# haoosz/FFR-Net

Hardware: AMD Instinct MI355X
Metric: face embeddings/sec (IR-SE50 + RecNet forward, 112x112 fp32) at batch 256 per GPU (higher is better)
Workload: dtype f32; 1 GPU; configs[2]: IR-SE50 + RecBlock (spatial+channel) forward, batch 256 per GPU, 112x112x3 fp32 -> f_new,f [512]; + all-gather of embeddings and pair cosine scores (112x96 of the BASELINE label cannot be embedded by the reference: BASELINE.md); batch_per_gpu=256, global_batch=256, parallelism=image-sharded x1, RCCL all-gather of embeddings

## Files before the change

ffr-net_amd/csrc/elementwise.hip:

```cpp
#include "device_util.h"
#include "ffr_kernels.h"

namespace ffr {

#define STEM_PIX 64
#define STEM_STEPS 8
#define STEM_TLD 36
template <bool U8>
__global__ __launch_bounds__(256) void k_stem(const float* __restrict__ x, const unsigned char* __restrict__ xu8,
                                             const unsigned char* __restrict__ flip, const float* __restrict__ w,
                                             const float* __restrict__ bias, const float* __restrict__ slope,
                                             float* __restrict__ out, int N, int H, int W,
                                             const float* __restrict__ x2, int n_split,
                                             const unsigned char* __restrict__ xu8b) {
    __shared__ __attribute__((aligned(16))) float patch[STEM_PIX * 28];
    __shared__ __attribute__((aligned(16))) float otile[4 * 32 * STEM_TLD];
    __shared__ float lut[U8 ? 257 : 1];
    const int tid = threadIdx.x;
    if constexpr (U8) {
        lut[tid] = __fdiv_rn(__fsub_rn(__fdiv_rn((float)tid, 255.0f), 0.5f), 0.5f);
        if (tid == 0) lut[256] = 0.f;
    }
    const int lane = tid & 63, wave = tid >> 6;
    const int mt = wave >> 1, nt = wave & 1;
// ... 270 lines not shown
                          int N, int Ho, int Wo, int C, int stride, hipStream_t stream) {
    const long long total4 = (long long)N * Ho * Wo * (C >> 2);
    const int cq = C >> 2;
    int shift = 0;
    while ((1 << shift) < cq) ++shift;
    if ((1 << shift) != cq || total4 >= 0x7fffffffLL || C % 4) return hipErrorInvalidValue;
    unsigned blocks = (unsigned)((total4 + 255) / 256);
    if (blocks > 8192) blocks = 8192;
    hipLaunchKernelGGL(k_combine, dim3(blocks), dim3(256), 0, stream, res, scale, sc, x, out, (unsigned)(Ho * Wo), (unsigned)Wo, C, stride,
                       (unsigned)total4, shift);
    return hipGetLastError();
}

__global__ __launch_bounds__(256) void k_affine(const float* __restrict__ x, const float* __restrict__ s,
                                               const float* __restrict__ t, float* __restrict__ y, int C,
                                               long long total4) {
    const int cq = C >> 2;
    for (long long idx = (long long)blockIdx.x * 256 + threadIdx.x; idx < total4; idx += (long long)gridDim.x * 256) {
        const int c4 = (int)(idx % cq) * 4;
        const f32x4 v = *reinterpret_cast<const f32x4*>(x + idx * 4);
        const f32x4 sv = *reinterpret_cast<const f32x4*>(s + c4);
        const f32x4 tv = *reinterpret_cast<const f32x4*>(t + c4);
        *reinterpret_cast<f32x4*>(y + idx * 4) = v * sv + tv;
    }
}

hipError_t launch_affine(const float* x, const float* s, const float* t, float* y, int M, int C, hipStream_t stream) {
    const long long total4 = (long long)M * (C >> 2);
    unsigned blocks = (unsigned)((total4 + 255) / 256);
    if (blocks > 4096) blocks = 4096;
    hipLaunchKernelGGL(k_affine, dim3(blocks), dim3(256), 0, stream, x, s, t, y, C, total4);
    return hipGetLastError();
}

__global__ __launch_bounds__(256) void k_head_finish(const float* __restrict__ partial, int splits, int N, int C,
                                                    const float* __restrict__ bias, float* __restrict__ f) {
    __shared__ float s_red[4];
    const int n = blockIdx.x, tid = threadIdx.x;
    float v[2];
    float ss = 0.f;
#pragma unroll
    for (int e = 0; e < 2; ++e) {
        const int c = tid + e * 256;
        float s = bias ? bias[c] : 0.f;
        for (int k = 0; k < splits; ++k) s += partial[((size_t)k * N + n) * C + c];
        v[e] = s;
// ... 219 lines not shown
```

ffr-net_amd/csrc/engine.cpp:

```cpp
#include "engine_internal.h"

using namespace ffr;
using namespace ffr_eng;

namespace ffr_eng {

std::string g_err = "";

int fail(ffr_handle* h, int code, const char* fmt, ...) {
    char buf[512];
    va_list ap;
    va_start(ap, fmt);
    vsnprintf(buf, sizeof buf, fmt, ap);
    va_end(ap);
    if (h) h->err = buf; else g_err = buf;
    return code;
}

struct PlanLayer { ConvW* L; std::string name; int net; };

std::vector<PlanLayer> plan_layers(const ffr_handle* hc) {
    ffr_handle* h = const_cast<ffr_handle*>(hc);
    std::vector<PlanLayer> v;
    if (h->enc_loaded)
// ... 29 lines not shown
    lay(measure);
    RC(grow(h, b, measure.off, what));
    Arena a(b.p);
    lay(a);
    return FFR_OK;
}

static int featmap_to_x(ffr_handle* h, const Work& w, const float* featmap_nchw, int N, hipStream_t st) {
    HIPCK(h, launch_nchw_to_nhwc(featmap_nchw, w.X, 512, N, 49, 512, st));
    return FFR_OK;
}

static int embed_tail(ffr_handle* h, const float* x, const U8In* u8, int N, float* f_new, float* f, hipStream_t st) {
    Work w;
    RC(ensure_arena_encoder(h, N, 112, 112, &w));
    RC(run_encoder(h, w, x, N, 112, 112, w.X, f, st, u8));
    return run_recnet(h, w, N, f_new, nullptr, st);
}

extern "C" {

const char* ffr_version(void) { return "ffrnet-hip 0.1 (gfx950)"; }

const char* ffr_last_error(const ffr_handle* h) { return h ? h->err.c_str() : g_err.c_str(); }

int ffr_create(ffr_handle** out, int device) {
    if (!out) return fail(nullptr, FFR_ERR_ARG, "ffr_create: out is null");
    *out = nullptr;
    int count = 0;
    if (hipGetDeviceCount(&count) != hipSuccess || count <= 0)
        return fail(nullptr, FFR_ERR_HIP, "no HIP device available (this library has no CPU fallback)");
    if (device < 0 || device >= count) return fail(nullptr, FFR_ERR_ARG, "device %d out of range (%d devices)", device, count);
// ... 937 lines not shown
    L.cin = L.cin_pad = d->cin_pad; L.cout = d->cout_store; L.cout_pad = d->cout_pad; L.R = d->R; L.S = d->S;
    L.stride = d->stride; L.pad = d->pad; L.pad_mode = d->pad_mode; L.border = d->border_bias;
    L.w = (float*)d->w; L.bias = (float*)d->bias; L.slope = (float*)d->slope;
    struct Planes { void* p = nullptr; ~Planes() { if (p) hipFree(p); } } planes;
    if (d->flags & 2) {
        if (!h->opt.igemm_split) return fail(h, FFR_ERR_STATE, "ffr_op_conv: flags bit1 asks for the split form, but option igemm_split is 0");
        const size_t nw = (size_t)d->cout_pad * d->R * d->S * d->cin_pad;
        HIPCK(h, hipMalloc(&planes.p, nw * 3 * sizeof(unsigned short)));
        HIPCK(h, launch_split_weights(d->w, (unsigned short*)planes.p, nw, (hipStream_t)stream));
        L.w3 = (unsigned short*)planes.p;
    }
    ConvCall c = conv_call(w);
    c.x = d->x; c.N = d->N; c.H = d->H; c.W = d->W; c.in_pitch = d->in_pitch; c.resid = d->resid; c.res_pitch = d->res_pitch;
    c.out = d->out; c.out_pitch = d->out_pitch; c.out_coff = d->out_coff; c.cout_store = d->cout_store; c.flags = d->flags & 1;
    c.tile = d->tile;
    const int rc = run_conv(h, L, c, (hipStream_t)stream);
    if (planes.p) hipStreamSynchronize((hipStream_t)stream);
    return rc;
}

int ffr_op_conv3x3(ffr_handle* h, const float* x, int N, int H, int W, int cin, const float* w_host,
                   const float* bias_host, const float* slope_host, int cout, int pad_mode, int use_wino,
                   const float* resid, float* out, void* stream) {
    FFR_DEVICE_SCOPE(h); RC(check_fwd(h, false, false, N));
    if (!x || !w_host || !bias_host || !out || cin % 32 || cout % 4 || cin <= 0 || cout <= 0)
        return fail(h, FFR_ERR_ARG, "ffr_op_conv3x3: bad arguments (cin %% 32, cout %% 4)");
    if (use_wino < 0 || use_wino > 5) return fail(h, FFR_ERR_ARG, "ffr_op_conv3x3: use_wino must be 0..5");
    hipStream_t st = (hipStream_t)stream;
    Work w;
    RC(ensure_arena(h, N > 8 ? N : 8, 112, 112, &w));
// ... 89 lines not shown
    for (int i = 0; i < *n && i < cap; ++i) out[i] = h->conv_log[i];
    return FFR_OK;
}

int ffr_plan_igemm_host(long long M, int cout_pad, int nkt, int nbatch, int force_tile, int min_units, int split, int count,
                        int* tile, int* nblocks, int* granule) {
    if (M < 1 || cout_pad < 64 || cout_pad % 64 || nkt < 1 || nbatch < 1 || min_units < 1 || count < 1 || !tile || !nblocks || !granule ||
        force_tile < 0 || force_tile > IGEMM_NTILES)
        return FFR_ERR_ARG;
    if (force_tile) {
        int bm, bn;
        igemm_tile_shape(force_tile, &bm, &bn);
        if (cout_pad % bn) return FFR_ERR_ARG;
    }
    for (int i = 0; i < count; ++i) plan_igemm(M + i, cout_pad, nkt, nbatch, force_tile, min_units, &tile[i], &nblocks[i], &granule[i], split != 0);
    return FFR_OK;
}

int ffr_plan_conv_host(int cin, int cout, int R, int stride, int pad, int pad_mode, int has_wino, int has_wu3, int has_w3,
                       int has_mixed, int N, int H, int W, int in_pitch, int out_pitch, int out_coff, int cout_store,
                       int res_pitch, int num_cus, int force, long long* out) {
    if (cin < 1 || cout < 1 || R < 1 || stride < 1 || pad < 0 || N < 1 || H < 1 || W < 1 || num_cus < 1 || force < -1 || force > 5 || !out)
        return FFR_ERR_ARG;
    static float mark[16];
    ffr_handle fh;
    fh.num_cus = num_cus;
    fh.side = (hipStream_t)(void*)&mark[15];
    ConvW L;
    L.cin = cin; L.cin_pad = round_up(cin, 32); L.cout = cout; L.cout_pad = round_up(cout, 64);
    L.R = R; L.S = R; L.stride = stride; L.pad = pad; L.pad_mode = pad_mode;
// ... 66 lines not shown
```

ffr-net_amd/csrc/engine_internal.h:

```cpp
#pragma once
#include <hip/hip_runtime.h>

#include <algorithm>
#include <chrono>
#include <cmath>
#include <cstdarg>
#include <cstdio>
#include <cstdlib>
#include <cstring>
#include <initializer_list>
#include <map>
#include <string>
#include <vector>

#include "../../include/ffrnet.h"
#include "../../include/ffrnet_train.h"
#include "ffr_kernels.h"

namespace ffr_eng {

using namespace ffr;

struct TrainState;

// ... 242 lines not shown

Work layout(const Options& opt, char* base, int N, int H, int W);
inline ConvCall conv_call(const Work& w, ConvForce force = ConvForce::Auto) {
    ConvCall c{};
    c.partial = w.partial; c.partial_cap = w.partial_cap; c.tickets = w.tickets; c.tickets_cap = w.tickets_cap;
    c.winoV = w.winoV; c.winoM = w.winoM; c.wino_cap = w.wino_cap; c.force = force;
    return c;
}
int grow(ffr_handle* h, DevBuf& b, size_t need_bytes, const char* what, bool zeroed = false);
int ensure_arena(ffr_handle* h, int N, int H, int W, Work* w);
int ensure_arena_encoder(ffr_handle* h, int N, int H, int W, Work* w);
struct U8In { const unsigned char* img; const unsigned char* flip; const unsigned char* img2 = nullptr; };
int run_trunk(ffr_handle* h, const Work& w, const float* x_nchw, int N, int H, int W, int n_blocks, hipStream_t st,
              float** out_ptr, int* oh, int* ow, int* oc, const U8In* u8 = nullptr, const float* x2 = nullptr, int n_split = 0);
int run_encoder(ffr_handle* h, const Work& w, const float* x, int N, int H, int W, float* featmap_nhwc, float* f,
                hipStream_t st, const U8In* u8 = nullptr, const float* x2 = nullptr, int n_split = 0);
struct RecDebug { float *ss_space, *M_space, *feat_space, *feat_channel_raw, *feat_channel, *ss_channel0, *M_channel0; int image = 0; };
int conv_rec(ffr_handle* h, const Work& w, const ConvW& L, const float* x, int in_pitch, const float* resid,
             int res_pitch, float* out, int out_pitch, int out_coff, int flags, int N, hipStream_t st);
int run_recnet(ffr_handle* h, const Work& w, int N, float* f_new, const RecDebug* dbg, hipStream_t st);
int check_fwd(ffr_handle* h, bool need_enc, bool need_rec, int N);
int gemm_rows(ffr_handle* h, const Work& w, const float* A, int a_pitch, int K_pad, const float* W, const float* bias,
              int N_pad, float* out, int out_pitch, long long rows, const float* resid, int res_pitch, int flags,
              hipStream_t st);
int gemm_batched(ffr_handle* h, const Work& w, const float* A, long long a_bstride, int K_pad, const float* W,
                 long long w_bstride, int N_pad, float* out, int out_pitch, long long out_bstride, int M, int nbatch,
                 hipStream_t st);
void train_free(ffr_handle* h);

}
```

ffr-net_amd/csrc/ffr_kernels.h:

```cpp
#pragma once
#include <hip/hip_runtime.h>
#include <stdint.h>
#include <type_traits>

#ifdef FFR_TRACE
#define FFR_TRACE_ON(p) ((p) != nullptr)
#else
#define FFR_TRACE_ON(p) false
#endif

namespace ffr {

struct ConvTail {
    const float* bias;
    const float* slope;
    const float* resid;
    float* out;
    float* tile_sums;
    int cout_pad;
    int cout_store;
    int out_pitch, out_coff, res_pitch;
    int border_bias;
    int flags;
};
// ... 2 lines not shown
    const float* x;
    const float* w;
    ConvTail tail;
    const float* zero;
    float* partial;
    int* tickets;
    unsigned long long* trace;
    int N, H, W, Ho, Wo, in_pitch, cin_pad, R, S, stride, pad, pad_mode;
    int M, KK, nkt, granule;
    int nbatch;
    long long x_bstride, w_bstride, out_bstride;
    int mtiles, ntiles;
    const unsigned short* w3;
    long long w3_pstride;
};
enum { IGEMM_TILE_128x128 = 1, IGEMM_TILE_128x64 = 2, IGEMM_TILE_64x64 = 3, IGEMM_TILE_256x64 = 4,
       IGEMM_NTILES = 4 };
struct IgemmTile { int bm, bn, wm, wn, wm_split, wn_split; };
constexpr IgemmTile IGEMM_TILES[IGEMM_NTILES + 1] = {
    {0, 0, 0, 0, 0, 0}, {128, 128, 2, 2, 4, 1}, {128, 64, 2, 2, 4, 1}, {64, 64, 2, 2, 2, 2}, {256, 64, 4, 1, 4, 1}};
template <typename F>
inline auto igemm_tile_dispatch(int tile, F&& f) -> decltype(f(std::integral_constant<int, IGEMM_TILE_128x128>{})) {
    switch (tile) {
        case IGEMM_TILE_128x128: return f(std::integral_constant<int, IGEMM_TILE_128x128>{});
        case IGEMM_TILE_128x64: return f(std::integral_constant<int, IGEMM_TILE_128x64>{});
        case IGEMM_TILE_64x64: return f(std::integral_constant<int, IGEMM_TILE_64x64>{});
        case IGEMM_TILE_256x64: return f(std::integral_constant<int, IGEMM_TILE_256x64>{});
        default: return {};
    }
}
// ... 103 lines not shown
hipError_t launch_combine_in_mixed(const float* res, const float* scale, const float* sh, float* out, float* V, int N, int H, int W,
                                   int C, hipStream_t stream);

hipError_t launch_mfma_probe(int iters, int blocks, unsigned long long* stamps, float* sink, hipStream_t stream);

hipError_t launch_stem(const float* x_nchw, const unsigned char* xu8, const unsigned char* flip, const float* w27x64,
                       const float* bias, const float* slope, float* out, int N, int H, int W, hipStream_t stream,
                       const float* x2 = nullptr, int n_split = 0, const unsigned char* xu8b = nullptr);
int se_slices(int N, int HW);
hipError_t launch_se(const float* res, int N, int HW, int C, const float* fc1, const float* fc2,
                     float* scale, float* part, hipStream_t stream);
hipError_t launch_se_fc(const float* part, int N, int S, int HW, int C, const float* fc1, const float* fc2, float* scale,
                        hipStream_t stream);
hipError_t launch_combine(const float* res, const float* scale, const float* sc, const float* x,
                          float* out, int N, int Ho, int Wo, int C, int stride, hipStream_t stream);
hipError_t launch_affine(const float* x, const float* s, const float* t, float* y, int M, int C,
                         hipStream_t stream);
hipError_t launch_head_finish(const float* partial, int splits, int N, int C, const float* bias,
                              float* f, hipStream_t stream);
hipError_t launch_nhwc_to_nchw(const float* in, int in_pitch, float* out, int N, int P, int C,
                               hipStream_t stream);
hipError_t launch_nchw_to_nhwc(const float* in, float* out, int out_pitch, int N, int P, int C,
                               hipStream_t stream);
hipError_t launch_copy_slice(const float* in, float* out, int M, int C, int pitch, int coff,
                             hipStream_t stream);
hipError_t launch_cosine(const float* a, const float* b, int n, int dim, float* score,
                         hipStream_t stream);
int absdiff_scratch_floats();
hipError_t launch_absdiff_max(const float* a, int a_pitch, const float* b, int b_pitch, int rows, int cols, float* part,
                              float* out, hipStream_t stream);

hipError_t launch_row_norms(const float* x, long long n, float* norms, hipStream_t stream);
// ... 105 lines not shown
```

ffr-net_amd/csrc/forward.cpp:

```cpp
#include "engine_internal.h"

namespace ffr_eng {


Work layout(const Options& opt, char* base, int N, int H, int W) {
    Arena a(base);
    Work w{};
    const size_t S0 = (size_t)N * H * W * 64;
    const size_t hw16 = (size_t)(H / 16) * (W / 16);
    w.bufA = a.take(S0);
    w.bufB = a.take(S0 / 4);
    w.t1 = a.take(S0);
    w.res = a.take(S0 / 4);
    w.sc = a.take(S0 / 8);
    w.scale = a.take((size_t)N * 512);
    w.se_part = a.take((size_t)N * 32 * 512);
    w.trunk_bn = a.take((size_t)N * hw16 * 512);
    w.partial_cap = (size_t)1024 * 2 * 128 * 128 / 2 + 4096;
    w.partial = a.take(w.partial_cap);
    {
        auto tiles = [&](int div) { return (size_t)N * ((H / div + 3) / 4) * ((W / div + 3) / 4); };
        size_t cap = 36 * tiles(2) * 128;
        if (36 * tiles(1) * 64 > cap) cap = 36 * tiles(1) * 64;
        if (36 * tiles(4) * 256 > cap) cap = 36 * tiles(4) * 256;
// ... 83 lines not shown
            c1.wino_stage = 1;
        if (v_ready) { c1.wino_stage = 2; c1.v_chunked = !v_mixed; c1.v_mixed = v_mixed; }
        const ConvPlan p1 = plan_conv(h, b.c1, c1);
        const bool chained = c1.wino_stage == 1 && p1.path == ConvPlan::Unfused;
        RC(run_conv(h, b.c1, c1, p1, st));
        if (chained) {
            Scope s(h, st, FFR_KC_WINO, 0, 4.0 * 72.0 * Tt * b.c1.cout_pad);
            if (h->conv_rec) note(FFR_CP_WINO_OUT_IN, (int)Tt, ((ch + 3) / 4) * ((cw + 3) / 4));
            HIPCK(h, launch_wino_out_in(w.winoM, b.c1.bias, b.c1.slope, w.winoV, N, ch, cw, b.c1.cout_pad, b.c1.border, st));
        }
        ConvCall c2 = conv_call(w);
        c2.x = w.t1; c2.N = N; c2.H = ch; c2.W = cw; c2.in_pitch = b.depth;
        c2.out = w.res; c2.out_pitch = b.depth; c2.cout_store = b.depth;
        if (chained) c2.wino_stage = 2;
        const int tiles = ((ho + 3) / 4) * ((wo + 3) / 4);
        if (b.fc1 && b.stride == 1 && tiles <= h->opt.se_maxtiles && (size_t)tiles * b.depth <= (size_t)32 * 512 && b.c2.cout_pad == b.depth)
            c2.tile_sums = w.se_part;
        const ConvPlan p2 = plan_conv(h, b.c2, c2);
        const bool pooled = c2.tile_sums && p2.path != ConvPlan::Direct;
        RC(run_conv(h, b.c2, c2, p2, st));
        const float* se_scale = nullptr;
        if (b.fc1) {
            const double e = (double)N * ho * wo * b.depth;
            Scope s(h, st, FFR_KC_SE, e + 4.0 * N * b.depth * (b.depth / 16), 4.0 * e);
            if (pooled) {
                if (h->conv_rec) note(FFR_CP_SE_TILES, ho * wo, tiles);
                HIPCK(h, launch_se_fc(w.se_part, N, tiles, ho * wo, b.depth, b.fc1, b.fc2, w.scale, st));
            } else {
                if (h->conv_rec) note(FFR_CP_SE_POOL, ho * wo, se_slices(N, ho * wo));
                HIPCK(h, launch_se(w.res, N, ho * wo, b.depth, b.fc1, b.fc2, w.scale, w.se_part, st));
            }
            se_scale = w.scale;
        }
        const float* scp = nullptr;
        if (b.has_sc) {
            ConvCall cs = conv_call(w);
            cs.x = cur; cs.N = N; cs.H = ch; cs.W = cw; cs.in_pitch = b.cin;
            cs.out = w.sc; cs.out_pitch = b.depth; cs.cout_store = b.depth;
            RC(run_conv(h, b.sc, cs, st));
            scp = w.sc;
        }
        ConvPlan next;
// ... 13 lines not shown
            if (h->conv_rec) note(FFR_CP_COMBINE_IN_C, ho * wo, tiles, b.stride, scp != nullptr, se_scale != nullptr);
            HIPCK(h, launch_combine_in_c(w.res, se_scale, scp ? scp : cur, nxt, w.winoV, N, ho, wo, b.depth, st));
        } else {
            Scope s(h, st, FFR_KC_COMBINE, 2.0 * e, 12.0 * e);
            if (h->conv_rec) note(FFR_CP_COMBINE, ho * wo, tiles, b.stride, scp != nullptr, se_scale != nullptr);
            HIPCK(h, launch_combine(w.res, se_scale, scp, cur, nxt, N, ho, wo, b.depth, b.stride, st));
        }
        float* t = cur; cur = nxt; nxt = t;
        ch = ho; cw = wo; cc = b.depth;
    }
    *out_ptr = cur; *oh = ch; *ow = cw; *oc = cc;
    return FFR_OK;
}

int run_encoder(ffr_handle* h, const Work& w, const float* x, int N, int H, int W, float* featmap_nhwc, float* f,
                hipStream_t st, const U8In* u8, const float* x2, int n_split) {
    float* t; int oh, ow, oc;
    RC(run_trunk(h, w, x, N, H, W, (int)h->blocks.size(), st, &t, &oh, &ow, &oc, u8, x2, n_split));
    const int P = oh * ow;
    if (featmap_nhwc) {
        Scope s(h, st, FFR_KC_HEAD, 2.0 * N * P * 512, 8.0 * N * P * 512);
        HIPCK(h, launch_affine(t, h->bn_s, h->bn_t, featmap_nhwc, N * P, 512, st));
    }
    if (f) {
        if (P != 49) return fail(h, FFR_ERR_UNSUPPORTED, "output_layer needs a 7x7 trunk map (112x112 input)");
        ConvCall c = conv_call(w);
        c.x = t; c.N = N; c.H = 1; c.W = 1; c.in_pitch = 25088;
        c.out = w.scale; c.out_pitch = 512; c.cout_store = 512;
        RC(run_conv(h, h->fc, c, st));
        Scope s(h, st, FFR_KC_HEAD, 3.0 * N * 512, 8.0 * N * 512);
        HIPCK(h, launch_head_finish(w.scale, 1, N, 512, nullptr, f, st));
    }
    return FFR_OK;
}


int conv_rec(ffr_handle* h, const Work& w, const ConvW& L, const float* x, int in_pitch, const float* resid,
// ... 16 lines not shown
    HIPCK(h, hipFree(dbuf));
    double ph[6] = {0, 0, 0, 0, 0, 0}; int cnt = 0;
    for (int b = 0; b < N * rb; ++b) {
        const unsigned long long* q = &tr[(size_t)b * 8];
        if (!q[6]) continue;
        for (int i = 0; i < 6; ++i) ph[i] += (double)(q[i + 1] - q[i]);
        ++cnt;
    }
    fprintf(stderr, "[wf trace] k_channel_path, %d images x %d row blocks: per block (wave 0) transpose+norms %.0f | G on MFMA %.0f | first linear %.0f | "
                    "two 32x32 affines %.0f | sigmoid(W8 h) @ X on MFMA %.0f | stores %.0f cyc\n", N, rb, ph[0] / cnt, ph[1] / cnt, ph[2] / cnt, ph[3] / cnt,
            ph[4] / cnt, ph[5] / cnt);
    return FFR_OK;
}
#endif

int run_recnet(ffr_handle* h, const Work& w, int N, float* f_new, const RecDebug* dbg, hipStream_t st) {
    const int M = N * 49;
    {
        Scope s(h, st, FFR_KC_LAYOUT, 0, 16.0 * M * 512);
        HIPCK(h, launch_copy_slice(w.X, w.bufS, M, 512, 576, 0, st));
        HIPCK(h, launch_copy_slice(w.X, w.bufM, M, 512, 1536, 1024, st));
    }
    {
        Scope s(h, st, FFR_KC_SELFSIM, 2.0 * N * 49 * 49 * 512, 4.0 * N * (49 * 512 + 49 * 49));
        HIPCK(h, launch_selfsim_space(w.X, w.bufS, 576, dbg ? dbg->ss_space : nullptr, N, st));
    }
    {
        const double fl = 2.0 * N * (512.0 * 512 * 49 + 512.0 * (561 * 32 + 5 * 32 * 512) + 512.0 * 512 * 49);
        Scope s(h, st, FFR_KC_CHANNEL, fl, 4.0 * N * (49 * 512 * 3));
        const int rb = plan_channel_rows(N, h->num_cus, h->opt.channel_rows);
        if (!rb) return fail(h, FFR_ERR_ARG, "channel_rows is 0 (auto), 1, 2 or 4");
        if (h->conv_rec) {
            ffr_conv_launch r{};
// ... 61 lines not shown
```

ffr-net_amd/csrc/igemm.hip:

```cpp
#include "conv_tail.h"
#include "ffr_kernels.h"
#include "igemm_core.h"

#include <utility>

namespace ffr {

template <int BM, int BN, int WARPS_M, int WARPS_N, int PAD_MODE, bool SPLIT = false>
__global__ __launch_bounds__(256) void k_igemm(const IgemmArgs a) {
    constexpr int WM = BM / WARPS_M, WN = BN / WARPS_N;
    constexpr int TM = WM / 32, TN = WN / 32;
    constexpr int A_PT = BM / 32;
    constexpr int B_PT = SPLIT ? 3 * (BN / 64) : BN / 32;
    constexpr int STAGE_FLOATS = igemm_stage_floats(BM, BN, SPLIT);
    static_assert(WARPS_M * WARPS_N == 4, "4 waves");
    extern __shared__ __attribute__((aligned(16))) float smem[];
    int* s_cls = reinterpret_cast<int*>(smem + igemm_cls_offset(BM, BN, SPLIT));
    float* s_bias = smem + igemm_bias_offset(BM, BN, SPLIT);

    const ConvTail& e = a.tail;
    const int wave = __builtin_amdgcn_readfirstlane(threadIdx.x >> 6);
    const int wm = wave / WARPS_N, wn = wave % WARPS_N;
    const int HoWo = a.Ho * a.Wo;

// ... 301 lines not shown
#pragma unroll
                    for (int k = 0; k < 8; ++k)
                        if (bb + k <= b_hi) sum += v[k];
                }
                *reinterpret_cast<f32x4*>(sC + ml * LDC + ecol) = sum;
            }
        }
    }
    if (finish) {
        const int n = n0 + ecol;
        const bool vec = ((e.out_pitch | e.out_coff | e.res_pitch) & 3) == 0 && n + 4 <= e.cout_store && !(e.flags & 1);
        const f32x4 slope4 = tail_slope4(e.slope, n);
        const f32x4 bias0 = *reinterpret_cast<const f32x4*>(e.bias + n);
        constexpr int NP = BM / RPP;
        constexpr int BATCH = NP < 4 ? NP : 4;
        auto finish_tile = [&]<bool BORDER, bool RESID>() {
            f32x4 rs[BATCH], rn[BATCH];
            const int mrow = m0 + erow;
            float* optr = ob + (size_t)mrow * e.out_pitch + e.out_coff + n;
            const size_t ostep = (size_t)RPP * e.out_pitch;
            const float* rptr = RESID ? e.resid + (size_t)mrow * e.res_pitch + n : nullptr;
            const size_t rstep = (size_t)RPP * e.res_pitch;
            auto load_resid = [&](f32x4* dstv, int p0) {
#pragma unroll
                for (int k = 0; k < BATCH; ++k) {
                    dstv[k] = (f32x4){0.f, 0.f, 0.f, 0.f};
                    if (mrow + (p0 + k) * RPP < a.M) dstv[k] = *reinterpret_cast<const f32x4*>(rptr + (size_t)(p0 + k) * rstep);
                }
            };
            if (RESID) load_resid(rs, 0);
#pragma unroll
            for (int p0 = 0; p0 < NP; p0 += BATCH) {
                if (RESID && p0 + BATCH < NP) load_resid(rn, p0 + BATCH);
#pragma unroll
                for (int k = 0; k < BATCH; ++k) {
                    const int ml = (p0 + k) * RPP + erow;
                    f32x4 v = *reinterpret_cast<const f32x4*>(sC + ml * LDC + ecol);
                    if (BORDER) v += *reinterpret_cast<const f32x4*>(s_bias + s_cls[ml] * BN + ecol);
                    else v += bias0;
#pragma unroll
                    for (int c = 0; c < 4; ++c) v[c] = v[c] >= 0.f ? v[c] : v[c] * slope4[c];
                    if (RESID) v += rs[k];
                    if (m0 + ml < a.M) *reinterpret_cast<f32x4*>(optr) = v;
                    optr += ostep;
                }
                if (RESID) {
#pragma unroll
                    for (int k = 0; k < BATCH; ++k) rs[k] = rn[k];
                }
            }
        };
        if (vec) {
            if (e.border_bias) {
                if (e.resid) finish_tile.template operator()<true, true>();
                else finish_tile.template operator()<true, false>();
            } else {
                if (e.resid) finish_tile.template operator()<false, true>();
                else finish_tile.template operator()<false, false>();
            }
        } else {
#pragma unroll 1
            for (int p = 0; p < NP; ++p) {
                const int ml = p * RPP + erow;
                const int m = m0 + ml;
                if (m >= a.M) continue;
                f32x4 v = *reinterpret_cast<const f32x4*>(sC + ml * LDC + ecol);
                v += e.border_bias ? *reinterpret_cast<const f32x4*>(s_bias + s_cls[ml] * BN + ecol) : bias0;
#pragma unroll
                for (int c = 0; c < 4; ++c) {
                    if (n + c < e.cout_store) {
                        float x = prelu<PRELU_SELECT>(v[c], slope4[c]);
                        x = tail_end1(x, e.resid != nullptr, [&] { return e.resid[(size_t)m * e.res_pitch + n + c]; }, e.flags);
                        ob[(size_t)m * e.out_pitch + e.out_coff + n + c] = x;
                    }
                }
            }
        }
    }
    if (FFR_TRACE_ON(a.trace)) { const unsigned long long t = __builtin_amdgcn_s_memtime(); tr_acc[3] += t - tr_t; tr_t = t; }
    }
    if (FFR_TRACE_ON(a.trace) && threadIdx.x == 0) {
        unsigned long long* t = a.trace + (size_t)blockIdx.x * 8;
        t[0] = tr_acc[0]; t[1] = tr_acc[1]; t[2] = tr_acc[2]; t[3] = tr_acc[3]; t[4] = tr_seg;
        t[5] = tr_rt0; t[6] = __builtin_amdgcn_s_memrealtime(); t[7] = (tr_acc[4] << 32) | (tr_acc[5] & 0xffffffffull);
    }
}

static const void* igemm_kernel(int tile, int pad_mode, bool split) {
    return igemm_tile_dispatch(tile, [&](auto t) -> const void* {
// ... 6 lines not shown
hipError_t igemm_init() {
    for (int i = 0; i < IGEMM_NTILES * 4; ++i) {
        const int tile = 1 + i / 4, split = i & 1;
        const hipError_t e = hipFuncSetAttribute(igemm_kernel(tile, (i >> 1) & 1, split), hipFuncAttributeMaxDynamicSharedMemorySize,
                                                 igemm_lds_bytes(IGEMM_TILES[tile].bm, IGEMM_TILES[tile].bn, split));
        if (e != hipSuccess) return e;
    }
    return hipSuccess;
}

hipError_t launch_igemm(const IgemmArgs& a, int tile, int nblocks, hipStream_t stream) {
    const bool split = a.w3 != nullptr;
    const void* kernel = igemm_kernel(tile, a.pad_mode, split);
    if (!kernel || nblocks <= 0) return hipErrorInvalidValue;
    if (split && a.nbatch != 1) return hipErrorInvalidValue;
    void* args[] = {const_cast<IgemmArgs*>(&a)};
    return hipLaunchKernel(kernel, dim3((unsigned)nblocks, 1, 1), dim3(256), args,
                           igemm_lds_bytes(IGEMM_TILES[tile].bm, IGEMM_TILES[tile].bn, split), stream);
}

__global__ void k_split_weights(const float* __restrict__ w, unsigned short* __restrict__ planes, size_t n) {
    for (size_t i = (size_t)blockIdx.x * blockDim.x + threadIdx.x; i < n; i += (size_t)gridDim.x * blockDim.x) {
        float r = w[i];
#pragma unroll
        for (int p = 0; p < 3; ++p) {
            const unsigned short h = (unsigned short)(cvt_pk_bf16(r, 0.f) & 0xffffu);
            planes[(size_t)p * n + i] = h;
            r -= __builtin_bit_cast(float, (unsigned)h << 16);
        }
    }
// ... 10 lines not shown
```

ffr-net_amd/native.py:

```python
import ctypes as C
import os

import torch

from . import align as _align

_HERE = os.path.dirname(os.path.abspath(__file__))
_LIB = None

KCLASS_NAMES = ['conv_igemm', 'stem', 'se', 'combine', 'head', 'selfsim', 'channel',
                'space', 'layout', 'score', 'wino', 'wino_fused', 'wgrad',
                'train_bn', 'train_loss', 'train_optim', 'train_xform', 'train_elem']


class NativeLibraryMissing(RuntimeError):
    pass


class TensorDesc(C.Structure):
    _fields_ = [('name', C.c_char_p), ('data', C.c_void_p), ('ndim', C.c_int32),
                ('shape', C.c_int64 * 4)]


class MemStats(C.Structure):
# ... 5 lines not shown

class KClassStat(C.Structure):
    _fields_ = [('launches', C.c_int64), ('ms', C.c_double), ('flops', C.c_double),
                ('bytes', C.c_double), ('flops_executed', C.c_double), ('flops_useful', C.c_double)]


class ConvDesc(C.Structure):
    _fields_ = [('x', C.c_void_p), ('N', C.c_int), ('H', C.c_int), ('W', C.c_int),
                ('in_pitch', C.c_int), ('cin_pad', C.c_int),
                ('w', C.c_void_p), ('bias', C.c_void_p), ('slope', C.c_void_p),
                ('resid', C.c_void_p), ('res_pitch', C.c_int),
                ('out', C.c_void_p), ('out_pitch', C.c_int), ('out_coff', C.c_int),
                ('cout_store', C.c_int), ('cout_pad', C.c_int),
                ('R', C.c_int), ('S', C.c_int), ('stride', C.c_int), ('pad', C.c_int),
                ('pad_mode', C.c_int), ('border_bias', C.c_int), ('flags', C.c_int),
                ('tile', C.c_int), ('splitk', C.c_int)]


class LayerInfo(C.Structure):
    _fields_ = [('name', C.c_char * 64), ('net', C.c_int), ('arith', C.c_int), ('sensitivity', C.c_double)]


class WgradLaunch(C.Structure):
    _fields_ = [('name', C.c_char * 48)] + [(f, C.c_int) for f in (
        'path', 'rows', 'cout_pad', 'Ng', 'nbatch', 'nkt', 'splits', 'kt_per_split', 'full_tiles', 'tail_splits', 'tail_kt',
        'accumulate')]


class Conv3x3Desc(C.Structure):
    _fields_ = [('x', C.c_void_p), ('N', C.c_int), ('H', C.c_int), ('W', C.c_int), ('cin', C.c_int), ('in_pitch', C.c_int),
                ('w_host', C.c_void_p), ('bias_host', C.c_void_p), ('slope_host', C.c_void_p), ('cout', C.c_int),
# ... 79 lines not shown
    ('ffr_calibrate', C.c_int, [_P, _P, _P, C.c_int, C.c_int, C.c_int, C.c_double, C.POINTER(C.c_double), _P]),
    ('ffr_memory_stats', C.c_int, [_P, _P]),
    ('ffr_split_planes_host', C.c_int, [_P, C.c_longlong, _P]),
    ('ffr_set_option', C.c_int, [_P, C.c_char_p, C.c_longlong]),
    ('ffr_get_option', C.c_int, [_P, C.c_char_p, C.POINTER(C.c_longlong)]),
    ('ffr_probe_mfma_peak', C.c_int, [_P, C.c_int, C.POINTER(C.c_double), C.POINTER(C.c_double), _P]),
    ('ffr_profile_enable', C.c_int, [_P, C.c_int]),
    ('ffr_profile_read', C.c_int, [_P, C.POINTER(KClassStat)]),
    ('ffr_op_conv', C.c_int, [_P, C.POINTER(ConvDesc), _P]),
    ('ffr_op_conv3x3', C.c_int, [_P, _P, C.c_int, C.c_int, C.c_int, C.c_int, _P, _P, _P, C.c_int, C.c_int, C.c_int, _P, _P, _P]),
    ('ffr_op_conv3x3_ex', C.c_int, [_P, C.POINTER(Conv3x3Desc), _P]),
    ('ffr_conv_plan_record', C.c_int, [_P, C.c_int]),
    ('ffr_conv_plan_read', C.c_int, [_P, C.POINTER(ConvLaunch), C.c_int, C.POINTER(C.c_int)]),
    ('ffr_plan_igemm_host', C.c_int, [C.c_longlong] + [C.c_int] * 7 + [_P, _P, _P]),
    ('ffr_plan_conv_host', C.c_int, [C.c_int] * 20 + [_P]),
    ('ffr_encoder_trunk_nhwc', C.c_int, [_P, _P, C.c_int, C.c_int, C.c_int, C.c_int, _P, _P]),
    ('ffr_plan_channel_rows_host', C.c_int, [C.c_int, C.c_int, C.c_int, _P]),
    ('ffr_recnet_debug', C.c_int, [_P, _P, C.c_int, _P, _P, _P, _P, _P, _P, _P, C.c_int, _P]),
    ('ffr_op_convlayer_train', C.c_int, [_P, _P, C.c_int, C.c_int, C.c_int, C.c_int, _P, _P, _P, _P, _P, _P, _P, _P, _P, _P, _P]),
    ('ffr_train_init', C.c_int, [_P, C.POINTER(TensorDesc), C.c_int]),
    ('ffr_train_info', C.c_int, [_P, C.POINTER(_P), C.POINTER(_P), C.POINTER(C.c_size_t), C.POINTER(C.c_longlong),
                                 C.POINTER(C.c_int)]),
    ('ffr_train_get', C.c_int, [_P, C.c_int, C.c_char_p, _P, C.c_size_t]),
    ('ffr_train_set', C.c_int, [_P, C.c_int, C.c_char_p, _P, C.c_size_t]),
    ('ffr_train_zero_grad', C.c_int, [_P, _P]),
    ('ffr_train_forward', C.c_int, [_P, C.c_int, _P, _P, C.c_int, C.c_int, _P, _P, _P, _P, _P, _P, _P, _P]),
    ('ffr_train_backward', C.c_int, [_P, C.c_int, _P, _P, _P, _P, _P, _P, _P, _P]),
    ('ffr_train_adam_step', C.c_int, [_P, C.c_double, C.c_double, C.c_double, C.c_double, C.c_double, C.c_double, _P]),
    ('ffr_train_debug_copy', C.c_int, [_P, C.c_int, C.c_char_p, _P, C.c_size_t]),
    ('ffr_train_option', C.c_int, [_P, C.c_char_p, C.c_int]),
# ... 731 lines not shown

    def profile_read(self):
        arr = (KClassStat * len(KCLASS_NAMES))()
        self._ck(self.lib.ffr_profile_read(self._h, arr))
        return {KCLASS_NAMES[i]: dict(launches=int(arr[i].launches), ms=arr[i].ms,
                                      flops=arr[i].flops, bytes=arr[i].bytes, flops_executed=arr[i].flops_executed,
                                      flops_useful=arr[i].flops_useful)
                for i in range(len(KCLASS_NAMES))}

    def op_conv(self, **kw):
        d = ConvDesc()
        for k, v in kw.items():
            if isinstance(v, torch.Tensor):
                v = v.data_ptr()
            elif v is None:
                v = 0 if k not in ('x', 'w', 'bias', 'slope', 'resid', 'out') else None
            setattr(d, k, v)
        self._call(self.lib.ffr_op_conv, C.byref(d))

    def op_conv3x3(self, x_nhwc, w, bias, slope=None, pad_mode=0, use_wino=True, resid=None):
        self._tensor(x_nhwc, 'x')
        x_nhwc = x_nhwc.contiguous()
        n, hh, ww, cin = x_nhwc.shape
        wh = w.detach().float().cpu().contiguous()
        bh = bias.detach().float().cpu().contiguous()
        sh = slope.detach().float().cpu().contiguous() if slope is not None else None
        out = self._empty(n, hh, ww, wh.size(0))
        self._call(self.lib.ffr_op_conv3x3, _ptr(x_nhwc), n, hh, ww, cin, _ptr(wh), _ptr(bh), _ptr(sh), wh.size(0), pad_mode,
                   int(use_wino), _ptr(resid.contiguous() if resid is not None else None), _ptr(out))
        return out

# ... 278 lines not shown
```

include/ffrnet.h:

```cpp
#ifndef FFRNET_H
#define FFRNET_H

#include <stddef.h>
#include <stdint.h>

#ifdef __cplusplus
extern "C" {
#endif

typedef struct ffr_handle ffr_handle;

typedef enum {
    FFR_OK = 0,
    FFR_ERR_ARG = -1,
    FFR_ERR_STATE = -2,
    FFR_ERR_KEY = -3,
    FFR_ERR_HIP = -4,
    FFR_ERR_NOMEM = -5,
    FFR_ERR_UNSUPPORTED = -6
} ffr_status;

typedef struct {
    const char*  name;
    const float* data;
// ... 146 lines not shown
    size_t wf_split_weight_bytes;
    long long wf_split_launches;
} ffr_mem_stats;
int ffr_memory_stats(const ffr_handle* h, ffr_mem_stats* out);
int ffr_split_planes_host(const double* w, long long n, unsigned short* planes);
int ffr_probe_mfma_peak(ffr_handle* h, int iters, double* tflops, double* clock_ghz, void* stream);
int ffr_profile_read(ffr_handle* h, ffr_kclass_stat* out );

typedef struct {
    const float* x; int N, H, W, in_pitch, cin_pad;
    const float* w; const float* bias; const float* slope;
    const float* resid; int res_pitch;
    float* out; int out_pitch, out_coff, cout_store, cout_pad;
    int R, S, stride, pad, pad_mode, border_bias, flags;
    int tile, splitk;
} ffr_conv_desc;
int ffr_op_conv(ffr_handle* h, const ffr_conv_desc* d, void* stream);

int ffr_op_conv3x3(ffr_handle* h, const float* x_nhwc, int N, int H, int W, int cin,
                   const float* w_host, const float* bias_host, const float* slope_host, int cout,
                   int pad_mode, int use_wino, const float* resid_nhwc, float* out_nhwc, void* stream);

typedef struct {
    const float* x; int N, H, W, cin, in_pitch;
    const float* w_host; const float* bias_host; const float* slope_host; int cout;
    const float* in_scale_host; const float* in_shift_host;
    const float* resid; int res_pitch;
    float* out; int out_pitch, out_coff, cout_store;
    int pad_mode, use_wino, flags;
    float* tile_sums;
// ... 3 lines not shown
enum { FFR_CP_DIRECT = 0, FFR_CP_FUSED = 1, FFR_CP_UNFUSED_STREAM = 2, FFR_CP_UNFUSED_IGEMM = 3, FFR_CP_MIXED = 4, FFR_CP_TAIL_SPLIT = 5,
       FFR_CP_CHANNEL = 6, FFR_CP_SE_POOL = 7, FFR_CP_SE_TILES = 8, FFR_CP_COMBINE = 9, FFR_CP_COMBINE_IN_C = 10,
       FFR_CP_COMBINE_IN_MIXED = 11, FFR_CP_WINO_OUT_IN = 12 };
typedef struct ffr_conv_launch {
    int path, images, rows;
    int tile, nblocks, granule, nkt, tiles, cut, split;
    int phased, half_n, block_tiles;
    int n_main, side;
    int stride, conv_shortcut, se_scale;
} ffr_conv_launch;
int ffr_conv_plan_record(ffr_handle* h, int on);
int ffr_conv_plan_read(ffr_handle* h, ffr_conv_launch* out, int cap, int* n);

int ffr_plan_igemm_host(long long M, int cout_pad, int nkt, int nbatch, int force_tile, int min_units, int split, int count,
                        int* tile, int* nblocks, int* granule);
int ffr_plan_conv_host(int cin, int cout, int R, int stride, int pad, int pad_mode, int has_wino, int has_wu3, int has_w3,
                       int has_mixed, int N, int H, int W, int in_pitch, int out_pitch, int out_coff, int cout_store,
                       int res_pitch, int num_cus, int force, long long* out);

int ffr_plan_channel_rows_host(int N, int num_cus, int forced, int* row_blocks);

int ffr_encoder_trunk_nhwc(ffr_handle* h, const float* x_nchw, int N, int H, int W,
                           int n_blocks, float* out_nhwc, void* stream);

int ffr_recnet_debug(ffr_handle* h, const float* featmap_nchw, int N,
                     float* ss_space, float* M_space, float* feat_space,
                     float* feat_channel_raw, float* feat_channel, float* ss_channel0, float* M_channel0,
                     int image, void* stream);

#ifdef __cplusplus
// ... 4 lines not shown
```

Measured before the change: 18310 embeddings/s.

## Fuse SE pooling into igemm epilogue and write RecNet slices from BN affine

The implicit-GEMM conv epilogue now accumulates per-image channel sums into tile_sums slots, so SE blocks on the direct/igemm path can skip the separate SE pooling pass over the residual map. Separately, the final BN affine kernel writes its output straight into the RecNet S and M buffers, which removes two copy_slice launches. In exchange the epilogue does extra LDS reductions and a barrier, and the affine kernel issues extra scattered stores.

```diff
diff --git a/ffr-net_amd/csrc/elementwise.hip b/ffr-net_amd/csrc/elementwise.hip
--- a/ffr-net_amd/csrc/elementwise.hip
+++ b/ffr-net_amd/csrc/elementwise.hip
@@ -308,22 +308,33 @@
 
 __global__ __launch_bounds__(256) void k_affine(const float* __restrict__ x, const float* __restrict__ s,
                                                const float* __restrict__ t, float* __restrict__ y, int C,
-                                               long long total4) {
+                                               long long total4, float* __restrict__ y1, int pitch1, int coff1,
+                                               float* __restrict__ y2, int pitch2, int coff2) {
     const int cq = C >> 2;
     for (long long idx = (long long)blockIdx.x * 256 + threadIdx.x; idx < total4; idx += (long long)gridDim.x * 256) {
         const int c4 = (int)(idx % cq) * 4;
         const f32x4 v = *reinterpret_cast<const f32x4*>(x + idx * 4);
         const f32x4 sv = *reinterpret_cast<const f32x4*>(s + c4);
         const f32x4 tv = *reinterpret_cast<const f32x4*>(t + c4);
-        *reinterpret_cast<f32x4*>(y + idx * 4) = v * sv + tv;
-    }
-}
-
-hipError_t launch_affine(const float* x, const float* s, const float* t, float* y, int M, int C, hipStream_t stream) {
+        const f32x4 r = v * sv + tv;
+        *reinterpret_cast<f32x4*>(y + idx * 4) = r;
+        if (y1 || y2) {
+            const long long m = idx / cq;
+            if (y1) *reinterpret_cast<f32x4*>(y1 + m * pitch1 + coff1 + c4) = r;
+            if (y2) *reinterpret_cast<f32x4*>(y2 + m * pitch2 + coff2 + c4) = r;
+        }
+    }
+}
+
+hipError_t launch_affine(const float* x, const float* s, const float* t, float* y, int M, int C, hipStream_t stream,
+                         const AffineSlice* y1, const AffineSlice* y2) {
     const long long total4 = (long long)M * (C >> 2);
+    for (const AffineSlice* e : {y1, y2})
+        if (e && (!e->out || ((e->pitch | e->coff) & 3) || e->coff + C > e->pitch)) return hipErrorInvalidValue;
     unsigned blocks = (unsigned)((total4 + 255) / 256);
     if (blocks > 4096) blocks = 4096;
-    hipLaunchKernelGGL(k_affine, dim3(blocks), dim3(256), 0, stream, x, s, t, y, C, total4);
+    hipLaunchKernelGGL(k_affine, dim3(blocks), dim3(256), 0, stream, x, s, t, y, C, total4, y1 ? y1->out : nullptr, y1 ? y1->pitch : 0,
+                       y1 ? y1->coff : 0, y2 ? y2->out : nullptr, y2 ? y2->pitch : 0, y2 ? y2->coff : 0);
     return hipGetLastError();
 }
 
diff --git a/ffr-net_amd/csrc/engine.cpp b/ffr-net_amd/csrc/engine.cpp
--- a/ffr-net_amd/csrc/engine.cpp
+++ b/ffr-net_amd/csrc/engine.cpp
@@ -67,8 +67,8 @@
 static int embed_tail(ffr_handle* h, const float* x, const U8In* u8, int N, float* f_new, float* f, hipStream_t st) {
     Work w;
     RC(ensure_arena_encoder(h, N, 112, 112, &w));
-    RC(run_encoder(h, w, x, N, 112, 112, w.X, f, st, u8));
-    return run_recnet(h, w, N, f_new, nullptr, st);
+    RC(run_encoder(h, w, x, N, 112, 112, w.X, f, st, u8, nullptr, 0, true));
+    return run_recnet(h, w, N, f_new, nullptr, st, true);
 }
 
 extern "C" {
@@ -1036,6 +1036,8 @@
     c.x = d->x; c.N = d->N; c.H = d->H; c.W = d->W; c.in_pitch = d->in_pitch; c.resid = d->resid; c.res_pitch = d->res_pitch;
     c.out = d->out; c.out_pitch = d->out_pitch; c.out_coff = d->out_coff; c.cout_store = d->cout_store; c.flags = d->flags & 1;
     c.tile = d->tile;
+    if (d->tile_sums && d->resid) return fail(h, FFR_ERR_ARG, "ffr_op_conv: tile_sums come from launches without a residual");
+    c.tile_sums = d->tile_sums;
     const int rc = run_conv(h, L, c, (hipStream_t)stream);
     if (planes.p) hipStreamSynchronize((hipStream_t)stream);
     return rc;
@@ -1155,6 +1157,19 @@
         if (cout_pad % bn) return FFR_ERR_ARG;
     }
     for (int i = 0; i < count; ++i) plan_igemm(M + i, cout_pad, nkt, nbatch, force_tile, min_units, &tile[i], &nblocks[i], &granule[i], split != 0);
+    return FFR_OK;
+}
+
+int ffr_igemm_sum_slots_host(int HW, int bm, int N, int* S, int* slot) {
+    if (HW < 1 || bm < 1 || N < 1 || !S || (long long)N * HW > 0x7fffffffLL) return FFR_ERR_ARG;
+    *S = igemm_sum_slots(HW, bm);
+    const int mtiles = (int)(((long long)N * HW + bm - 1) / bm);
+    if (slot)
+        for (int n = 0; n < N; ++n)
+            for (int mt = 0; mt < mtiles; ++mt) {
+                const bool has_rows = (long long)mt * bm < (long long)(n + 1) * HW && (long long)(mt + 1) * bm > (long long)n * HW;
+                slot[(size_t)n * mtiles + mt] = has_rows ? igemm_sum_slot(n, mt, HW, bm) : -1;
+            }
     return FFR_OK;
 }
 
diff --git a/ffr-net_amd/csrc/engine_internal.h b/ffr-net_amd/csrc/engine_internal.h
--- a/ffr-net_amd/csrc/engine_internal.h
+++ b/ffr-net_amd/csrc/engine_internal.h
@@ -280,11 +280,11 @@
 int run_trunk(ffr_handle* h, const Work& w, const float* x_nchw, int N, int H, int W, int n_blocks, hipStream_t st,
               float** out_ptr, int* oh, int* ow, int* oc, const U8In* u8 = nullptr, const float* x2 = nullptr, int n_split = 0);
 int run_encoder(ffr_handle* h, const Work& w, const float* x, int N, int H, int W, float* featmap_nhwc, float* f,
-                hipStream_t st, const U8In* u8 = nullptr, const float* x2 = nullptr, int n_split = 0);
+                hipStream_t st, const U8In* u8 = nullptr, const float* x2 = nullptr, int n_split = 0, bool rec_slices = false);
 struct RecDebug { float *ss_space, *M_space, *feat_space, *feat_channel_raw, *feat_channel, *ss_channel0, *M_channel0; int image = 0; };
 int conv_rec(ffr_handle* h, const Work& w, const ConvW& L, const float* x, int in_pitch, const float* resid,
              int res_pitch, float* out, int out_pitch, int out_coff, int flags, int N, hipStream_t st);
-int run_recnet(ffr_handle* h, const Work& w, int N, float* f_new, const RecDebug* dbg, hipStream_t st);
+int run_recnet(ffr_handle* h, const Work& w, int N, float* f_new, const RecDebug* dbg, hipStream_t st, bool x_slices_filled = false);
 int check_fwd(ffr_handle* h, bool need_enc, bool need_rec, int N);
 int gemm_rows(ffr_handle* h, const Work& w, const float* A, int a_pitch, int K_pad, const float* W, const float* bias,
               int N_pad, float* out, int out_pitch, long long rows, const float* resid, int res_pitch, int flags,
diff --git a/ffr-net_amd/csrc/ffr_kernels.h b/ffr-net_amd/csrc/ffr_kernels.h
--- a/ffr-net_amd/csrc/ffr_kernels.h
+++ b/ffr-net_amd/csrc/ffr_kernels.h
@@ -40,6 +40,8 @@
     const unsigned short* w3;
     long long w3_pstride;
 };
+__host__ __device__ inline int igemm_sum_slots(int HW, int bm) { return (HW + bm - 1) / bm + 1; }
+__host__ __device__ inline int igemm_sum_slot(int img, int mt, int HW, int bm) { return mt - (int)((long long)img * HW / bm); }
 enum { IGEMM_TILE_128x128 = 1, IGEMM_TILE_128x64 = 2, IGEMM_TILE_64x64 = 3, IGEMM_TILE_256x64 = 4,
        IGEMM_NTILES = 4 };
 struct IgemmTile { int bm, bn, wm, wn, wm_split, wn_split; };
@@ -173,8 +175,9 @@
                         hipStream_t stream);
 hipError_t launch_combine(const float* res, const float* scale, const float* sc, const float* x,
                           float* out, int N, int Ho, int Wo, int C, int stride, hipStream_t stream);
+struct AffineSlice { float* out; int pitch, coff; };
 hipError_t launch_affine(const float* x, const float* s, const float* t, float* y, int M, int C,
-                         hipStream_t stream);
+                         hipStream_t stream, const AffineSlice* y1 = nullptr, const AffineSlice* y2 = nullptr);
 hipError_t launch_head_finish(const float* partial, int splits, int N, int C, const float* bias,
                               float* f, hipStream_t stream);
 hipError_t launch_nhwc_to_nchw(const float* in, int in_pitch, float* out, int N, int P, int C,
diff --git a/ffr-net_amd/csrc/forward.cpp b/ffr-net_amd/csrc/forward.cpp
--- a/ffr-net_amd/csrc/forward.cpp
+++ b/ffr-net_amd/csrc/forward.cpp
@@ -121,18 +121,27 @@
         c2.out = w.res; c2.out_pitch = b.depth; c2.cout_store = b.depth;
         if (chained) c2.wino_stage = 2;
         const int tiles = ((ho + 3) / 4) * ((wo + 3) / 4);
-        if (b.fc1 && b.stride == 1 && tiles <= h->opt.se_maxtiles && (size_t)tiles * b.depth <= (size_t)32 * 512 && b.c2.cout_pad == b.depth)
-            c2.tile_sums = w.se_part;
         const ConvPlan p2 = plan_conv(h, b.c2, c2);
-        const bool pooled = c2.tile_sums && p2.path != ConvPlan::Direct;
+        int se_slots = 0;
+        if (b.fc1 && b.c2.cout_pad == b.depth) {
+            if (p2.path != ConvPlan::Direct) {
+                if (b.stride == 1 && tiles <= h->opt.se_maxtiles && (size_t)tiles * b.depth <= (size_t)32 * 512) se_slots = tiles;
+            } else if (p2.n_launch == 1 && !p2.refused) {
+                int bm, bn;
+                igemm_tile_shape(p2.launch[0].gemm.tile, &bm, &bn);
+                const int S = igemm_sum_slots(ho * wo, bm);
+                if (bm >= 128 && (size_t)S * b.depth <= (size_t)32 * 512) se_slots = S;
+            }
+        }
+        if (se_slots) c2.tile_sums = w.se_part;
         RC(run_conv(h, b.c2, c2, p2, st));
         const float* se_scale = nullptr;
         if (b.fc1) {
             const double e = (double)N * ho * wo * b.depth;
             Scope s(h, st, FFR_KC_SE, e + 4.0 * N * b.depth * (b.depth / 16), 4.0 * e);
-            if (pooled) {
-                if (h->conv_rec) note(FFR_CP_SE_TILES, ho * wo, tiles);
-                HIPCK(h, launch_se_fc(w.se_part, N, tiles, ho * wo, b.depth, b.fc1, b.fc2, w.scale, st));
+            if (se_slots) {
+                if (h->conv_rec) note(FFR_CP_SE_TILES, ho * wo, se_slots);
+                HIPCK(h, launch_se_fc(w.se_part, N, se_slots, ho * wo, b.depth, b.fc1, b.fc2, w.scale, st));
             } else {
                 if (h->conv_rec) note(FFR_CP_SE_POOL, ho * wo, se_slices(N, ho * wo));
                 HIPCK(h, launch_se(w.res, N, ho * wo, b.depth, b.fc1, b.fc2, w.scale, w.se_part, st));
@@ -176,13 +185,15 @@
 }
 
 int run_encoder(ffr_handle* h, const Work& w, const float* x, int N, int H, int W, float* featmap_nhwc, float* f,
-                hipStream_t st, const U8In* u8, const float* x2, int n_split) {
+                hipStream_t st, const U8In* u8, const float* x2, int n_split, bool rec_slices) {
     float* t; int oh, ow, oc;
     RC(run_trunk(h, w, x, N, H, W, (int)h->blocks.size(), st, &t, &oh, &ow, &oc, u8, x2, n_split));
     const int P = oh * ow;
+    if (rec_slices && (featmap_nhwc != w.X || P != 49)) return fail(h, FFR_ERR_ARG, "RecNet's slices are filled from a 7x7 featmap in the workspace's X only");
     if (featmap_nhwc) {
-        Scope s(h, st, FFR_KC_HEAD, 2.0 * N * P * 512, 8.0 * N * P * 512);
-        HIPCK(h, launch_affine(t, h->bn_s, h->bn_t, featmap_nhwc, N * P, 512, st));
+        const AffineSlice toS{w.bufS, 576, 0}, toM{w.bufM, 1536, 1024};
+        Scope s(h, st, FFR_KC_HEAD, 2.0 * N * P * 512, (rec_slices ? 16.0 : 8.0) * N * P * 512);
+        HIPCK(h, launch_affine(t, h->bn_s, h->bn_t, featmap_nhwc, N * P, 512, st, rec_slices ? &toS : nullptr, rec_slices ? &toM : nullptr));
     }
     if (f) {
         if (P != 49) return fail(h, FFR_ERR_UNSUPPORTED, "output_layer needs a 7x7 trunk map (112x112 input)");
@@ -229,9 +240,9 @@
 }
 #endif
 
-int run_recnet(ffr_handle* h, const Work& w, int N, float* f_new, const RecDebug* dbg, hipStream_t st) {
+int run_recnet(ffr_handle* h, const Work& w, int N, float* f_new, const RecDebug* dbg, hipStream_t st, bool x_slices_filled) {
     const int M = N * 49;
-    {
+    if (!x_slices_filled) {
         Scope s(h, st, FFR_KC_LAYOUT, 0, 16.0 * M * 512);
         HIPCK(h, launch_copy_slice(w.X, w.bufS, M, 512, 576, 0, st));
         HIPCK(h, launch_copy_slice(w.X, w.bufM, M, 512, 1536, 1024, st));
diff --git a/ffr-net_amd/csrc/igemm.hip b/ffr-net_amd/csrc/igemm.hip
--- a/ffr-net_amd/csrc/igemm.hip
+++ b/ffr-net_amd/csrc/igemm.hip
@@ -339,7 +339,19 @@
         const f32x4 bias0 = *reinterpret_cast<const f32x4*>(e.bias + n);
         constexpr int NP = BM / RPP;
         constexpr int BATCH = NP < 4 ? NP : 4;
-        auto finish_tile = [&]<bool BORDER, bool RESID>() {
+        const bool sums = e.tile_sums != nullptr;
+        f32x4 ts_acc = {0.f, 0.f, 0.f, 0.f};
+        int ts_rem = sums ? (m0 + erow) % HoWo : 0;
+        auto ts_add = [&](int ml, const f32x4& stored) {
+            ts_acc += stored;
+            ts_rem += RPP;
+            if (ts_rem >= HoWo || ml + RPP >= BM) {
+                *reinterpret_cast<f32x4*>(sC + ml * LDC + ecol) = ts_acc;
+                ts_acc = (f32x4){0.f, 0.f, 0.f, 0.f};
+                while (ts_rem >= HoWo) ts_rem -= HoWo;
+            }
+        };
+        auto finish_tile = [&]<bool BORDER, bool RESID, bool SUMS>() {
             f32x4 rs[BATCH], rn[BATCH];
             const int mrow = m0 + erow;
             float* optr = ob + (size_t)mrow * e.out_pitch + e.out_coff + n;
@@ -368,6 +380,7 @@
                     if (RESID) v += rs[k];
                     if (m0 + ml < a.M) *reinterpret_cast<f32x4*>(optr) = v;
                     optr += ostep;
+                    if (SUMS) ts_add(ml, m0 + ml < a.M ? v : (f32x4){0.f, 0.f, 0.f, 0.f});
                 }
                 if (RESID) {
 #pragma unroll
@@ -375,29 +388,57 @@
                 }
             }
         };
-        if (vec) {
+        if (vec && sums) {
+            if (e.border_bias) finish_tile.template operator()<true, false, true>();
+            else finish_tile.template operator()<false, false, true>();
+        } else if (vec) {
             if (e.border_bias) {
-                if (e.resid) finish_tile.template operator()<true, true>();
-                else finish_tile.template operator()<true, false>();
+                if (e.resid) finish_tile.template operator()<true, true, false>();
+                else finish_tile.template operator()<true, false, false>();
             } else {
-                if (e.resid) finish_tile.template operator()<false, true>();
-                else finish_tile.template operator()<false, false>();
+                if (e.resid) finish_tile.template operator()<false, true, false>();
+                else finish_tile.template operator()<false, false, false>();
             }
         } else {
 #pragma unroll 1
             for (int p = 0; p < NP; ++p) {
                 const int ml = p * RPP + erow;
                 const int m = m0 + ml;
-                if (m >= a.M) continue;
-                f32x4 v = *reinterpret_cast<const f32x4*>(sC + ml * LDC + ecol);
-                v += e.border_bias ? *reinterpret_cast<const f32x4*>(s_bias + s_cls[ml] * BN + ecol) : bias0;
-#pragma unroll
-                for (int c = 0; c < 4; ++c) {
-                    if (n + c < e.cout_store) {
-                        float x = prelu<PRELU_SELECT>(v[c], slope4[c]);
-                        x = tail_end1(x, e.resid != nullptr, [&] { return e.resid[(size_t)m * e.res_pitch + n + c]; }, e.flags);
-                        ob[(size_t)m * e.out_pitch + e.out_coff + n + c] = x;
+                f32x4 st4 = {0.f, 0.f, 0.f, 0.f};
+                if (m < a.M) {
+                    f32x4 v = *reinterpret_cast<const f32x4*>(sC + ml * LDC + ecol);
+                    v += e.border_bias ? *reinterpret_cast<const f32x4*>(s_bias + s_cls[ml] * BN + ecol) : bias0;
+#pragma unroll
+                    for (int c = 0; c < 4; ++c) {
+                        if (n + c < e.cout_store) {
+                            float x = prelu<PRELU_SELECT>(v[c], slope4[c]);
+                            x = tail_end1(x, e.resid != nullptr, [&] { return e.resid[(size_t)m * e.res_pitch + n + c]; }, e.flags);
+                            ob[(size_t)m * e.out_pitch + e.out_coff + n + c] = x;
+                            st4[c] = x;
+                        }
                     }
+                }
+                if (sums) ts_add(ml, st4);
+            }
+        }
+        if (sums) {
+            asm volatile("s_waitcnt lgkmcnt(0)\n\ts_barrier" ::: "memory");
+            const int S = igemm_sum_slots(HoWo, BM);
+            const int m_end = m0 + BM < a.M ? m0 + BM : a.M;
+            if (tid < BN) {
+                for (int img = m0 / HoWo; img * HoWo < m_end; ++img) {
+                    const int r0 = img * HoWo > m0 ? img * HoWo - m0 : 0;
+                    const int r1 = (img + 1) * HoWo - m0 < BM ? (img + 1) * HoWo - m0 : BM;
+                    float s = 0.f;
+                    for (int g = 0; g < RPP; ++g) {
+                        const int ml = r1 - 1 - ((r1 - 1 - g) & (RPP - 1));
+                        if (ml >= r0) s += sC[ml * LDC + tid];
+                    }
+                    const int slot = igemm_sum_slot(img, mt, HoWo, BM);
+                    float* dst = e.tile_sums + ((size_t)img * S + slot) * e.cout_pad + n0 + tid;
+                    *dst = s;
+                    if ((img + 1) * HoWo - m0 <= BM)
+                        for (int k = slot + 1; k < S; ++k) dst[(size_t)(k - slot) * e.cout_pad] = 0.f;
                 }
             }
         }
@@ -434,6 +475,7 @@
     const void* kernel = igemm_kernel(tile, a.pad_mode, split);
     if (!kernel || nblocks <= 0) return hipErrorInvalidValue;
     if (split && a.nbatch != 1) return hipErrorInvalidValue;
+    if (a.tail.tile_sums && (a.tail.resid || a.nbatch != 1)) return hipErrorInvalidValue;
     void* args[] = {const_cast<IgemmArgs*>(&a)};
     return hipLaunchKernel(kernel, dim3((unsigned)nblocks, 1, 1), dim3(256), args,
                            igemm_lds_bytes(IGEMM_TILES[tile].bm, IGEMM_TILES[tile].bn, split), stream);
diff --git a/ffr-net_amd/native.py b/ffr-net_amd/native.py
--- a/ffr-net_amd/native.py
+++ b/ffr-net_amd/native.py
@@ -43,7 +43,7 @@
                 ('cout_store', C.c_int), ('cout_pad', C.c_int),
                 ('R', C.c_int), ('S', C.c_int), ('stride', C.c_int), ('pad', C.c_int),
                 ('pad_mode', C.c_int), ('border_bias', C.c_int), ('flags', C.c_int),
-                ('tile', C.c_int), ('splitk', C.c_int)]
+                ('tile', C.c_int), ('splitk', C.c_int), ('tile_sums', C.c_void_p)]
 
 
 class LayerInfo(C.Structure):
@@ -153,6 +153,7 @@
     ('ffr_conv_plan_read', C.c_int, [_P, C.POINTER(ConvLaunch), C.c_int, C.POINTER(C.c_int)]),
     ('ffr_plan_igemm_host', C.c_int, [C.c_longlong] + [C.c_int] * 7 + [_P, _P, _P]),
     ('ffr_plan_conv_host', C.c_int, [C.c_int] * 20 + [_P]),
+    ('ffr_igemm_sum_slots_host', C.c_int, [C.c_int, C.c_int, C.c_int, _P, _P]),
     ('ffr_encoder_trunk_nhwc', C.c_int, [_P, _P, C.c_int, C.c_int, C.c_int, C.c_int, _P, _P]),
     ('ffr_plan_channel_rows_host', C.c_int, [C.c_int, C.c_int, C.c_int, _P]),
     ('ffr_recnet_debug', C.c_int, [_P, _P, C.c_int, _P, _P, _P, _P, _P, _P, _P, C.c_int, _P]),
@@ -914,7 +915,7 @@
             if isinstance(v, torch.Tensor):
                 v = v.data_ptr()
             elif v is None:
-                v = 0 if k not in ('x', 'w', 'bias', 'slope', 'resid', 'out') else None
+                v = 0 if k not in ('x', 'w', 'bias', 'slope', 'resid', 'out', 'tile_sums') else None
             setattr(d, k, v)
         self._call(self.lib.ffr_op_conv, C.byref(d))
 
diff --git a/include/ffrnet.h b/include/ffrnet.h
--- a/include/ffrnet.h
+++ b/include/ffrnet.h
@@ -184,6 +184,7 @@
     float* out; int out_pitch, out_coff, cout_store, cout_pad;
     int R, S, stride, pad, pad_mode, border_bias, flags;
     int tile, splitk;
+    float* tile_sums;
 } ffr_conv_desc;
 int ffr_op_conv(ffr_handle* h, const ffr_conv_desc* d, void* stream);
 
@@ -217,6 +218,7 @@
 
 int ffr_plan_igemm_host(long long M, int cout_pad, int nkt, int nbatch, int force_tile, int min_units, int split, int count,
                         int* tile, int* nblocks, int* granule);
+int ffr_igemm_sum_slots_host(int HW, int bm, int N, int* S, int* slot);
 int ffr_plan_conv_host(int cin, int cout, int R, int stride, int pad, int pad_mode, int has_wino, int has_wu3, int has_w3,
                        int has_mixed, int N, int H, int W, int in_pitch, int out_pitch, int out_coff, int cout_store,
                        int res_pitch, int num_cus, int force, long long* out);
```

Measured after the change: 18320 embeddings/s (median of 2 runs). About the same (+0.1%).
